# tzeitim/rogtk

Hardware: AMD Instinct MI355X
Metric: reads/s UMI score+cluster, 150 bp/12 bp UMI, 1→8 MI355X; % HBM roofline (higher is better)
Workload: dtype u32/f64

## Files before the change

rogtk_amd/csrc/cluster_kernels.hip:

```cpp
#include <hip/hip_ext.h>
#include <hipcub/hipcub.hpp>

#include <algorithm>
#include <cstdlib>
#include <map>
#include <mutex>

#include <atomic>
#include <thread>
#include <chrono>
#include <cstring>

#include "rogtk_internal.h"

namespace rogtk {
namespace {

constexpr int kBlock = 256;
constexpr int kMarkParts = 8;
constexpr int kMarkChunks = 256;
constexpr int kScanWords = 1024;
constexpr int kLocal8Words = 1024;
constexpr int kLocal8Cap = 8192;
constexpr int kLocal8BigCap = 16384;
// ... 1758 lines not shown
    if (rounds) {
        ++st.epoch;
        st.launched = launched;
        st.checked = checked;
        st.pending = true;
    }
    return ROGTK_OK;
}

int cluster_finish(const void* ws, hipStream_t s, int* redone) {
    if (redone) *redone = 0;
    std::lock_guard<std::mutex> lk(g_rs_mu);
    auto it = g_rs.find(ws);
    if (it == g_rs.end() || !it->second.pending) return ROGTK_OK;
    return finish_locked(ws, it->second, s, redone);
}

namespace {
int finish_locked(const void* ws, ResolveState& st, hipStream_t s, int* redone) {
    if (int rc = wait_published(st)) return rc;
    unsigned int* hflags = (unsigned int*)(st.hstats + kFlagsOff);
    const unsigned long long* hs = (const unsigned long long*)st.hstats;
    st.lcc_choice = hs[S_P0] == 8 ? (int)hs[S_LCAP] : 2;
    const bool redo = hs[S_REDO] != 0;
    const int scanned = st.launched + (st.checked ? 1 : 0);
    st.checked = false;
    if (!redo) {
        if (int z = first_zero(hflags, 0, scanned); z >= 0) {
            st.pending = false;
            st.deferred.on = false;
            st.rounds = z + 1;
            st.needed = st.rounds;
            return ROGTK_OK;
        }
    }
    if (redone) *redone = 1;
    WsPtrs p = ws_ptrs(st.cl, const_cast<uint8_t*>((const uint8_t*)ws));
    if (redo) {
        ProfScope prof(K_UNION, s);
        ROGTK_HIP_CHECK(hipMemsetAsync(p.stats + S_REDO, 0, 8, s));
        launch_local_cc(p.RT, st.cl.words, st.cl.L, p.f, p.UR, p.lroot, st.cl.rwords, st.cl.max_distinct, p.stats, s,
                        -1);
        ROGTK_HIP_CHECK(hipGetLastError());
        ROGTK_HIP_CHECK(hipMemsetAsync(p.flags, 0, kMaxRounds * sizeof(unsigned int), s));
        std::memset(hflags, 0, kMaxRounds * sizeof(unsigned int));
        st.launched = 0;
    }
    bool converged = false;
    while (!converged && st.launched < kMaxRounds) {
        const int to = std::min(st.launched + kRoundBatch, kMaxRounds);
        {
            ProfScope prof(K_UNION, s);
            if (int rc = enqueue_rounds(st.cl, p, st.launched, to, s)) return rc;
        }
        ROGTK_HIP_CHECK(hipMemcpyAsync(hflags + st.launched, p.flags + st.launched,
                                       (to - st.launched) * sizeof(unsigned int), hipMemcpyDeviceToHost, s));
        ROGTK_HIP_CHECK(hipStreamSynchronize(s));
        const int z = first_zero(hflags, st.launched, to);
        converged = z >= 0;
        if (converged) st.rounds = st.needed = z + 1;
        st.launched = to;
    }
    st.pending = false;
    ROGTK_REQUIRE(converged, ROGTK_E_HIP, "cluster: union rounds did not converge in %d rounds", kMaxRounds);
    if (int rc = enqueue_labels(st.cl, p, s, nullptr)) return rc;
    if (st.deferred.on) {
        st.deferred.on = false;
        return enqueue_assign(st.cl, p, st.word_labels ? 1 : st.exact ? 2 : 0, st.deferred.codes, st.deferred.regbits, st.deferred.n,
                              st.deferred.cid, s);
    }
    return ROGTK_OK;
}
}

int cluster_set_spec_rounds(int n) {
    ROGTK_REQUIRE(n >= 0 && n <= kMaxRounds, ROGTK_E_INVALID, "spec rounds %d outside 0..%d", n, kMaxRounds);
    g_spec_rounds.store(n == 0 ? kSpecRounds : n);
    g_spec_adaptive.store(n == 0);
    return ROGTK_OK;
}

int cluster_set_lookback_polls(int n) {
    ROGTK_REQUIRE(n >= -1, ROGTK_E_INVALID, "look-back polls %d < -1", n);
    g_lb_polls.store(n < 0 ? kLbMaxPolls : n);
    return ROGTK_OK;
}

int cluster_rounds(const void* ws, hipStream_t s, int* rounds) {
    if (int rc = cluster_finish(ws, s)) return rc;
    std::lock_guard<std::mutex> lk(g_rs_mu);
    auto it = g_rs.find(ws);
    *rounds = it == g_rs.end() ? 0 : it->second.rounds;
    return ROGTK_OK;
}

void cluster_release(const void* ws) {
    std::lock_guard<std::mutex> lk(g_rs_mu);
    auto it = g_rs.find(ws);
    if (it == g_rs.end()) return;
    if (it->second.hstats) {
        if (it->second.pending) (void)wait_published(it->second);
        hipHostFree(it->second.hstats);
    }
    g_rs.erase(it);
}

int launch_cluster_assign(const ClusterLayout& cl, const uint8_t* ws, const uint32_t* codes,
                          const uint64_t* regular_bits, int64_t n, uint32_t* cluster_id,
                          hipStream_t s, bool deferred) {
    if (!deferred)
        if (int rc = cluster_finish(ws, s)) return rc;
    WsPtrs p = ws_ptrs(cl, const_cast<uint8_t*>(ws));
    int wl = 0;
    {
        std::lock_guard<std::mutex> lk(g_rs_mu);
        auto it = g_rs.find(ws);
        if (it != g_rs.end()) {
            wl = it->second.word_labels ? 1 : it->second.exact ? 2 : 0;
            if (deferred && it->second.pending) {
                auto& d = it->second.deferred;
                d.on = true;
                d.codes = codes;
                d.regbits = regular_bits;
                d.n = n;
                d.cid = cluster_id;
            }
        }
    }
    return enqueue_assign(cl, p, wl, codes, regular_bits, n, cluster_id, s);
}

int cluster_assign_prepare(const ClusterLayout& cl, const uint8_t* ws, const uint32_t* codes,
                           const uint64_t* regular_bits, int64_t n, uint32_t* cluster_id, hipStream_t s,
                           bool deferred, AssignIn* a) {
    a->wlab = nullptr;
    a->wexc = nullptr;
    a->labelcode = nullptr;
    a->out = nullptr;
    if (!deferred)
        if (int rc = cluster_finish(ws, s)) return rc;
    bool wl = false;
    {
        std::lock_guard<std::mutex> lk(g_rs_mu);
        auto it = g_rs.find(ws);
        if (it != g_rs.end()) {
            wl = it->second.word_labels;
            if (deferred && it->second.pending) {
                auto& d = it->second.deferred;
                d.on = true;
                d.codes = codes;
                d.regbits = regular_bits;
                d.n = n;
                d.cid = cluster_id;
            }
        }
    }
    if (!wl || !cl.label_by_code) return ROGTK_OK;
    WsPtrs p = ws_ptrs(cl, const_cast<uint8_t*>(ws));
    a->wlab = p.wpref;
    a->wexc = p.G;
    a->labelcode = p.labelcode;
    a->out = cluster_id;
    return ROGTK_OK;
}

int launch_cluster_lookup(const ClusterLayout& cl, const uint8_t* ws, const uint64_t* q, int64_t nq, uint32_t* lab,
                          hipStream_t s) {
    if (nq <= 0) return ROGTK_OK;
    if (int rc = cluster_finish(ws, s)) return rc;
    WsPtrs p = ws_ptrs(cl, const_cast<uint8_t*>(ws));
    bool wl = false;
    {
        std::lock_guard<std::mutex> lk(g_rs_mu);
        auto it = g_rs.find(ws);
        if (it != g_rs.end()) wl = it->second.word_labels;
    }
    const uint32_t* wlab = wl ? p.wpref : nullptr;
    const uint64_t* wexc = wl ? p.G : nullptr;
    const int g = grid_for(nq, 4096);
    if (cl.label_by_code)
        hipLaunchKernelGGL(k_lookup<0>, dim3(g), dim3(kBlock), 0, s, q, nq, cl.nbits, p.labelcode, p.D, p.RT, wlab,
                           wexc, lab);
    else
        hipLaunchKernelGGL(k_lookup<1>, dim3(g), dim3(kBlock), 0, s, q, nq, cl.nbits, p.labelcode, p.ilab, p.RT, wlab,
                           wexc, lab);
    ROGTK_HIP_CHECK(hipGetLastError());
    return ROGTK_OK;
}

#ifndef ROGTK_ASSIGN_WGS
#define ROGTK_ASSIGN_WGS 2
#endif
#ifndef ROGTK_ASSIGN_G
#define ROGTK_ASSIGN_G 2
#endif
namespace {
int enqueue_assign(const ClusterLayout& cl, const WsPtrs& p, int labels, const uint32_t* codes,
                   const uint64_t* regular_bits, int64_t n, uint32_t* cluster_id, hipStream_t s) {
    if (n <= 0) return ROGTK_OK;
    const uint32_t* wlab = labels == 1 ? p.wpref : nullptr;
    const uint64_t* wexc = labels == 1 ? p.G : nullptr;
    ProfScope prof(K_ASSIGN, s, true);
    static const int64_t cap = [] {
        int dev = 0, cus = 0;
        if (hipGetDevice(&dev) != hipSuccess ||
            hipDeviceGetAttribute(&cus, hipDeviceAttributeMultiprocessorCount, dev) != hipSuccess || cus <= 0)
            cus = 256;
        return (int64_t)ROGTK_ASSIGN_WGS * cus;
    }();
    constexpr int kGroups = ROGTK_ASSIGN_G;
    const int g = grid_for((n + 4 * kGroups - 1) / (4 * kGroups), cap);
    if (labels == 2)
        hipExtLaunchKernelGGL((k_assign<2, kGroups>), dim3(g), dim3(kBlock), 0, s, prof.start(), prof.stop(), 0, codes,
                              regular_bits, n, p.labelcode, p.ilab, p.RT, wlab, wexc, cluster_id);
    else if (cl.label_by_code)
        hipExtLaunchKernelGGL((k_assign<0, kGroups>), dim3(g), dim3(kBlock), 0, s, prof.start(), prof.stop(), 0, codes,
                              regular_bits, n, p.labelcode, p.D, p.RT, wlab, wexc, cluster_id);
    else
        hipExtLaunchKernelGGL((k_assign<1, kGroups>), dim3(g), dim3(kBlock), 0, s, prof.start(), prof.stop(), 0, codes,
                              regular_bits, n, p.labelcode, p.ilab, p.RT, wlab, wexc, cluster_id);
    ROGTK_HIP_CHECK(hipGetLastError());
    return ROGTK_OK;
}
}



namespace {

constexpr int kPartBits = 8;
constexpr int kPartBlock = 512;

__global__ __launch_bounds__(kBlock) void k_mark_keys(const uint32_t* __restrict__ codes,
                                                      const uint64_t* __restrict__ regbits, int64_t n,
                                                      uint32_t* __restrict__ keys) {
    const int64_t i = (int64_t)blockIdx.x * kBlock + threadIdx.x;
    if (i >= n) return;
    const bool reg = (regbits[i >> 6] >> (i & 63)) & 1ull;
    keys[i] = reg ? codes[i] : 0xFFFFFFFFu;
}

__device__ int64_t wg_lower_bound(const uint32_t* __restrict__ a, int64_t n, uint64_t v) {
    int64_t lo = 0, hi = n;
    while (lo < hi) {
        const int64_t step = (hi - lo + kPartBlock - 1) / kPartBlock;
        const int64_t pos = lo + (int64_t)threadIdx.x * step;
        const bool less = pos < hi && (uint64_t)a[pos] < v;
        const int64_t cnt = __syncthreads_count(less);
        const int64_t nlo = cnt ? lo + (cnt - 1) * step + 1 : lo;
        const int64_t nhi = min(hi, lo + cnt * step);
        lo = nlo;
        hi = nhi;
    }
    return lo;
}

__global__ __launch_bounds__(kPartBlock) void k_part_bitmap(const uint32_t* __restrict__ sorted, int64_t n,
                                                            int two_l, uint64_t* __restrict__ bitmap) {
    extern __shared__ uint32_t lbits[];
    const int p = blockIdx.x;
    const int shift = two_l - kPartBits;
    const uint32_t pwords32 = (1u << shift) >> 5;
    for (uint32_t k = threadIdx.x; k < pwords32; k += kPartBlock) lbits[k] = 0;
    __shared__ int64_t range[2];
    const int64_t r0 = wg_lower_bound(sorted, n, (uint64_t)p << shift);
    const int64_t r1 = p + 1 == (1 << kPartBits) ? n : wg_lower_bound(sorted, n, (uint64_t)(p + 1) << shift);
    if (threadIdx.x == 0) {
        range[0] = r0;
        range[1] = r1;
    }
    __syncthreads();
    const uint32_t mask = (1u << shift) - 1u;
    constexpr int kUnroll = 8;
    const int64_t rend = range[1];
    for (int64_t i0 = range[0] + threadIdx.x; i0 < rend; i0 += (int64_t)kPartBlock * kUnroll) {
        uint32_t key[kUnroll];
#pragma unroll
        for (int u = 0; u < kUnroll; ++u) {
            const int64_t i = i0 + (int64_t)u * kPartBlock;
            key[u] = i < rend ? __builtin_nontemporal_load(sorted + i) : 0xFFFFFFFFu;
        }
#pragma unroll
        for (int u = 0; u < kUnroll; ++u) {
            if ((uint64_t)key[u] >> two_l) continue;
            const uint32_t c = key[u] & mask;
            atomicOr(&lbits[c >> 5], 1u << (c & 31));
        }
    }
    __syncthreads();
    uint64_t* out = bitmap + ((uint64_t)p << shift >> 6);
    for (uint32_t k = threadIdx.x; k < pwords32 / 2; k += kPartBlock)
        out[k] = (uint64_t)lbits[2 * k] | ((uint64_t)lbits[2 * k + 1] << 32);
}

#ifndef ROGTK_SLICE_BLOCK
#define ROGTK_SLICE_BLOCK 1024
#endif
constexpr int kSliceBlock = ROGTK_SLICE_BLOCK;
constexpr int kSliceChunks = 8;
#ifndef ROGTK_SLICE_LOG2
#define ROGTK_SLICE_LOG2 20
#endif
constexpr int kSliceLog2 = ROGTK_SLICE_LOG2;
constexpr int kSliceBits = 24 - kSliceLog2;
constexpr int kMaxSlices = 1 << kSliceBits;
constexpr int kBucketRows = 8192;
constexpr int kSegCap = kBucketRows * 4 / kMaxSlices;

__global__ __launch_bounds__(kSliceBlock) void k_slice_mark(const uint32_t* __restrict__ codes,
                                                            const uint64_t* __restrict__ regbits, int64_t n,
                                                            int slice_log2, int chunks, int64_t chunk_rows,
                                                            uint64_t* __restrict__ out, int64_t words,
                                                            const uint32_t* __restrict__ segs = nullptr,
                                                            const uint32_t* __restrict__ seglen = nullptr,
                                                            int nbuckets = 0, int bucket_rows = kBucketRows,
                                                            int seg_cap = kSegCap) {
    __shared__ uint32_t sbits[(1u << kSliceLog2) / 32];
    const int c = blockIdx.x % chunks, sl = blockIdx.x / chunks;
    const uint32_t sw32 = (1u << slice_log2) >> 5;
    for (uint32_t k = threadIdx.x; k < sw32; k += kSliceBlock) sbits[k] = 0;
    __syncthreads();
    const uint32_t smask = (1u << slice_log2) - 1u;
    int64_t r0 = (int64_t)c * chunk_rows, r1 = min(n, r0 + chunk_rows);
    if (segs) {
        const int b0 = (int)((int64_t)c * nbuckets / chunks), b1 = (int)((int64_t)(c + 1) * nbuckets / chunks);
        bool over = false;
        for (int b = b0 + (int)threadIdx.x; b < b1; b += kSliceBlock)
            over |= seglen[(int64_t)sl * nbuckets + b] > (uint32_t)seg_cap;
        r0 = (int64_t)b0 * bucket_rows;
        r1 = min(n, (int64_t)b1 * bucket_rows);
        if (!__syncthreads_or(over)) {
            constexpr int kSegInFlight = 8;
            constexpr int kWaves = kSliceBlock / 64;
            const int wave = threadIdx.x >> 6, lane = threadIdx.x & 63;
            for (int bb = b0 + wave; bb < b1; bb += kWaves * kSegInFlight) {
                uint32_t len[kSegInFlight];
                uint32_t mx = 0;
#pragma unroll
                for (int u = 0; u < kSegInFlight; ++u) {
                    const int b = bb + u * kWaves;
                    len[u] = b < b1 ? seglen[(int64_t)sl * nbuckets + b] : 0u;
                    mx = max(mx, len[u]);
                }
                for (uint32_t i = 4 * lane; i < mx; i += 256) {
                    uint4 v[kSegInFlight];
#pragma unroll
                    for (int u = 0; u < kSegInFlight; ++u) {
                        const uint32_t* seg = segs + ((int64_t)sl * nbuckets + bb + u * kWaves) * seg_cap;
                        v[u] = i < len[u] ? *reinterpret_cast<const uint4*>(seg + i) : make_uint4(0, 0, 0, 0);
                    }
#pragma unroll
                    for (int u = 0; u < kSegInFlight; ++u) {
                        const uint32_t cc[4] = {v[u].x, v[u].y, v[u].z, v[u].w};
#pragma unroll
                        for (int k = 0; k < 4; ++k)
                            if (i + k < len[u]) {
                                const uint32_t b2 = cc[k] & smask;
                                atomicOr(&sbits[b2 >> 5], 1u << (b2 & 31));
                            }
                    }
                }
            }
            r1 = r0;
        }
    }
    constexpr int kSliceUnroll = 8;
    constexpr int64_t kStep = 4 * (int64_t)kSliceBlock;
    for (int64_t rb = r0 + 4 * (int64_t)threadIdx.x; rb < r1; rb += kStep * kSliceUnroll) {
        uint4 v[kSliceUnroll];
        uint32_t reg[kSliceUnroll];
#pragma unroll
        for (int u = 0; u < kSliceUnroll; ++u) {
            const int64_t r = rb + u * kStep;
            reg[u] = 0;
            v[u] = make_uint4(0, 0, 0, 0);
            if (r + 4 <= r1) {
                v[u] = *reinterpret_cast<const uint4*>(codes + r);
                reg[u] = regbits ? (uint32_t)(regbits[r >> 6] >> (r & 63)) & 0xFu : 0xFu;
            } else if (r < r1) {
                v[u].x = codes[r];
                if (r + 1 < r1) v[u].y = codes[r + 1];
                if (r + 2 < r1) v[u].z = codes[r + 2];
                reg[u] = (regbits ? (uint32_t)(regbits[r >> 6] >> (r & 63)) & 0xFu : 0xFu) &
                         ((1u << (uint32_t)(r1 - r)) - 1u);
            }
        }
#pragma unroll
        for (int u = 0; u < kSliceUnroll; ++u) {
            const uint32_t cc[4] = {v[u].x, v[u].y, v[u].z, v[u].w};
#pragma unroll
            for (int k = 0; k < 4; ++k)
                if (((reg[u] >> k) & 1u) && (cc[k] >> slice_log2) == (uint32_t)sl) {
                    const uint32_t b = cc[k] & smask;
                    atomicOr(&sbits[b >> 5], 1u << (b & 31));
                }
        }
    }
    __syncthreads();
    uint64_t* o = out + (int64_t)c * words + (((int64_t)sl << slice_log2) >> 6);
    for (uint32_t k = threadIdx.x; k < sw32 / 2; k += kSliceBlock)
        o[k] = (uint64_t)sbits[2 * k] | ((uint64_t)sbits[2 * k + 1] << 32);
}

constexpr int kBucketThreads = 1024;
template <int kBucketRows, int kBucketThreads>
__global__ __launch_bounds__(kBucketThreads) void k_slice_bucket(const uint32_t* __restrict__ codes,
                                                         const uint64_t* __restrict__ regbits, int64_t n,
                                                         int slice_log2, int nslices, uint32_t* __restrict__ segs,
                                                         uint32_t* __restrict__ seglen, int nbuckets) {
    __shared__ unsigned int cnt[kMaxSlices], lbase[kMaxSlices + 1];
    constexpr int kSegCap = kBucketRows * 4 / kMaxSlices;
    __shared__ uint32_t stage[kBucketRows];
    const int t = threadIdx.x, lane = t & 63;
    if (t < kMaxSlices) cnt[t] = 0;
    __syncthreads();
    const int64_t row0 = (int64_t)blockIdx.x * kBucketRows;
    constexpr int kPer = kBucketRows / kBucketThreads / 4;
    uint32_t key[kPer * 4];
    uint32_t val[kPer * 4];
    uint32_t regs[kPer];
#pragma unroll
    for (int u = 0; u < kPer; ++u) {
        const int64_t r = row0 + 4 * ((int64_t)u * kBucketThreads + t);
        uint4 v = make_uint4(0, 0, 0, 0);
        uint32_t reg = 0;
        if (r + 4 <= n) {
            v = *reinterpret_cast<const uint4*>(codes + r);
            reg = regbits ? (uint32_t)(regbits[r >> 6] >> (r & 63)) & 0xFu : 0xFu;
        } else if (r < n) {
            v.x = codes[r];
            if (r + 1 < n) v.y = codes[r + 1];
            if (r + 2 < n) v.z = codes[r + 2];
            reg = (regbits ? (uint32_t)(regbits[r >> 6] >> (r & 63)) & 0xFu : 0xFu) & ((1u << (uint32_t)(n - r)) - 1u);
        }
        val[4 * u] = v.x;
        val[4 * u + 1] = v.y;
        val[4 * u + 2] = v.z;
        val[4 * u + 3] = v.w;
        regs[u] = reg;
    }
#pragma unroll
    for (int u = 0; u < kPer; ++u) {
#pragma unroll
        for (int k = 0; k < 4; ++k) {
            const uint32_t sl = val[4 * u + k] >> slice_log2;
            const bool ok = ((regs[u] >> k) & 1u) && sl < (uint32_t)nslices;
            uint64_t peers = __ballot(ok);
#pragma unroll
            for (int bit = 0; bit < kSliceBits; ++bit) {
                const uint64_t b = __ballot((sl >> bit) & 1u);
                peers &= ((sl >> bit) & 1u) ? b : ~b;
            }
            const int leader = peers ? __ffsll((long long)peers) - 1 : 0;
            unsigned int base = 0;
            if (ok && lane == leader) base = atomicAdd(&cnt[sl], (unsigned int)__popcll(peers));
            base = __shfl(base, leader);
            key[4 * u + k] = ok ? (sl << 16) | (base + (uint32_t)__popcll(peers & ((1ull << lane) - 1ull))) : kNone;
        }
    }
    __syncthreads();
    if (t < nslices) seglen[(int64_t)t * nbuckets + blockIdx.x] = cnt[t];
    if (t == 0) {
        unsigned int acc = 0;
        for (int k = 0; k < nslices; ++k) {
            lbase[k] = acc;
            acc += cnt[k];
        }
        lbase[nslices] = acc;
    }
    __syncthreads();
#pragma unroll
    for (int u = 0; u < kPer * 4; ++u) {
        const uint32_t kk = key[u];
        if (kk != kNone) stage[lbase[kk >> 16] + (kk & 0xFFFFu)] = val[u];
    }
    __syncthreads();
    const unsigned int total = lbase[nslices];
    for (unsigned int i = t; i < total; i += kBucketThreads) {
        const uint32_t c = stage[i];
        const uint32_t sl = c >> slice_log2;
        if (cnt[sl] <= (unsigned int)kSegCap) segs[((int64_t)sl * nbuckets + blockIdx.x) * kSegCap + (i - lbase[sl])] = c;
    }
}

__global__ __launch_bounds__(kBlock) void k_or_partials(const uint64_t* __restrict__ partials, int chunks,
                                                        int64_t words, uint64_t* __restrict__ out) {
    for (int64_t w = (int64_t)blockIdx.x * kBlock + threadIdx.x; w < words; w += (int64_t)gridDim.x * kBlock) {
        uint64_t v = 0;
        for (int c = 0; c < chunks; ++c) v |= __builtin_nontemporal_load(partials + (int64_t)c * words + w);
        out[w] = v;
    }
}

inline int slice_chunks(int64_t n) { return n >= (1 << 20) ? kSliceChunks : 1; }
inline bool slice_segments(int64_t n) { return n >= (1 << 20); }
inline int slices_of(int L) { return 1 << (2 * L - std::min(2 * L, kSliceLog2)); }
inline int64_t seg_buckets(int64_t n) { return (n + kBucketRows - 1) / kBucketRows; }
inline int64_t seg_bytes(int64_t n) {
    return ((int64_t)kMaxSlices * seg_buckets(n) * kSegCap * 4) + ((int64_t)kMaxSlices * seg_buckets(n) * 4 + 255) / 256 * 256;
}
inline bool slice_buckets_on() {
    static const bool on = [] {
        const char* e = getenv("ROGTK_SLICE_BUCKETS");
        return !(e && e[0] == '0');
    }();
    return on;
}

size_t part_sort_temp(int64_t n) {
    size_t tb = 0;
    hipcub::DeviceRadixSort::SortKeys(nullptr, tb, (const uint32_t*)nullptr, (uint32_t*)nullptr, (int)n, 0, 8);
    return tb;
}

}

namespace {
std::atomic<int> g_mark_method{0};
bool use_slices(int L) {
    const int m = g_mark_method.load();
    return L <= 12 && m != 1;
}
}

int cluster_set_mark_method(int m) {
    ROGTK_REQUIRE(m >= 0 && m <= 2, ROGTK_E_INVALID, "mark method %d outside 0..2", m);
    g_mark_method.store(m);
    return ROGTK_OK;
}

int cluster_mark_bitmap_temp(int64_t n, int L, int64_t* bytes) {
    ROGTK_REQUIRE(L >= 7 && L <= 13, ROGTK_E_UNSUPPORTED, "mark_bitmap needs umi_len 7..13, got %d", L);
    ROGTK_REQUIRE(n >= 0 && n < ((int64_t)1 << 31), ROGTK_E_INVALID, "n outside 0..2^31-1");
    const int64_t nn = std::max<int64_t>(n, 1);
    const int64_t sort_bytes = 2 * ((nn * 4 + 255) / 256 * 256) + (int64_t)part_sort_temp(nn) + 256;
    const int64_t words = ((int64_t)1 << (2 * L)) / 64;
    int64_t slice_bytes = 0;
    if (L <= 12 && slice_segments(nn)) {
        slice_bytes = slice_chunks(nn) > 1 ? (int64_t)slice_chunks(nn) * words * 8 : 0;
        if (slices_of(L) > 1) slice_bytes += seg_bytes(nn);
    }
    *bytes = std::max(sort_bytes, slice_bytes);
    return ROGTK_OK;
}

int launch_cluster_mark_bitmap(const uint32_t* codes, const uint64_t* regular_bits, int64_t n, int L,
                               uint64_t* bitmap, void* temp, int64_t temp_bytes, hipStream_t s) {
    return launch_cluster_mark_phase(codes, regular_bits, n, L, bitmap, temp, temp_bytes, 0, s);
}

int launch_cluster_mark_phase(const uint32_t* codes, const uint64_t* regular_bits, int64_t n, int L,
                              uint64_t* bitmap, void* temp, int64_t temp_bytes, int phase, hipStream_t s) {
    ROGTK_REQUIRE(phase >= 0 && phase <= 2, ROGTK_E_INVALID, "mark_bitmap: phase %d", phase);
    int64_t need = 0;
    if (int rc = cluster_mark_bitmap_temp(n, L, &need)) return rc;
    ROGTK_REQUIRE((temp || n == 0) && temp_bytes >= need, ROGTK_E_INVALID, "temp_bytes %lld < %lld", (long long)temp_bytes,
                  (long long)need);
    ProfScope prof(K_MARK, s);
    const int two_l = 2 * L;
    if (n == 0) {
        if (phase != 1) ROGTK_HIP_CHECK(hipMemsetAsync(bitmap, 0, ((size_t)1 << two_l) / 8, s));
        return ROGTK_OK;
    }
    ROGTK_REQUIRE(((uintptr_t)codes & 15u) == 0, ROGTK_E_INVALID, "mark_bitmap: codes must be 16-byte aligned");
    if (use_slices(L)) {
        const int slog = std::min(two_l, kSliceLog2);
        const int slices = 1 << (two_l - slog);
        const int chunks = slice_chunks(n);
        int64_t chunk_rows = (n + chunks - 1) / chunks;
        chunk_rows = (chunk_rows + 3) / 4 * 4;
        const int64_t words = ((int64_t)1 << two_l) / 64;
        uint64_t* dst = chunks > 1 ? (uint64_t*)temp : bitmap;
        const uint32_t* segs = nullptr;
        uint32_t* seglen = nullptr;
        const int nb = (int)seg_buckets(n);
        if (slice_segments(n) && slices > 1 && slices <= kMaxSlices && slice_buckets_on()) {
            segs = (const uint32_t*)((uint8_t*)temp + (chunks > 1 ? (int64_t)chunks * words * 8 : 0));
            seglen = (uint32_t*)((uint8_t*)segs + (int64_t)kMaxSlices * nb * kSegCap * 4);
            if (phase != 2)
                ROGTK_TIMED_LAUNCH(K_K_SLICE_BUCKET, (k_slice_bucket<kBucketRows, kBucketThreads>), dim3((unsigned)nb),
                                   dim3(kBucketThreads), 0, s, codes, regular_bits, n, slog, slices, (uint32_t*)segs,
                                   seglen, nb);
        }
        if (phase == 1) {
            ROGTK_HIP_CHECK(hipGetLastError());
            return ROGTK_OK;
        }
        ROGTK_TIMED_LAUNCH(K_K_SLICE_MARK, k_slice_mark, dim3((unsigned)(slices * chunks)), dim3(kSliceBlock), 0, s, codes, regular_bits,
                           n, slog, chunks, chunk_rows, dst, words, segs, (const uint32_t*)seglen, nb, kBucketRows, kSegCap);
        if (chunks > 1)
            ROGTK_TIMED_LAUNCH(K_K_OR_PARTIALS, k_or_partials, dim3(grid_for(words, 4096)), dim3(kBlock), 0, s, dst, chunks, words,
                               bitmap);
        ROGTK_HIP_CHECK(hipGetLastError());
        return ROGTK_OK;
    }
    if (phase == 1) return ROGTK_OK;
    const int64_t slab = (n * 4 + 255) / 256 * 256;
    uint32_t* keys_in = (uint32_t*)temp;
    uint32_t* keys_out = (uint32_t*)((uint8_t*)temp + slab);
    void* cub = (uint8_t*)temp + 2 * slab;
    const uint32_t* src = codes;
    if (regular_bits) {
        hipLaunchKernelGGL(k_mark_keys, dim3((unsigned)((n + kBlock - 1) / kBlock)), dim3(kBlock), 0, s, codes,
                           regular_bits, n, keys_in);
        src = keys_in;
    }
    size_t tb = part_sort_temp(n);
    ROGTK_HIP_CHECK(hipcub::DeviceRadixSort::SortKeys(cub, tb, src, keys_out, (int)n, two_l - kPartBits, two_l, s));
    const size_t lds = ((size_t)1 << (two_l - kPartBits)) / 8;
    hipLaunchKernelGGL(k_part_bitmap, dim3(1u << kPartBits), dim3(kPartBlock), lds, s, keys_out, n, two_l, bitmap);
    ROGTK_HIP_CHECK(hipGetLastError());
    return ROGTK_OK;
}

}

#ifdef ROGTK_LCC_TIMING
extern "C" int rogtk_debug_lcc_clock(unsigned long long* out8) {
    if (hipMemcpyFromSymbol(out8, HIP_SYMBOL(rogtk::g_lcc_clk), 64) != hipSuccess) return 1;
    const unsigned long long z[8] = {0, 0, 0, 0, 0, 0, 0, 0};
    return hipMemcpyToSymbol(HIP_SYMBOL(rogtk::g_lcc_clk), z, 64) == hipSuccess ? 0 : 1;
}
#endif
```

Baseline: 36.75 billion.

## Replace capped slice segments with compact 16-bit bucketed runs and per-slice mark

```diff
diff --git a/rogtk_amd/csrc/cluster_kernels.hip b/rogtk_amd/csrc/cluster_kernels.hip
--- a/rogtk_amd/csrc/cluster_kernels.hip
+++ b/rogtk_amd/csrc/cluster_kernels.hip
@@ -2084,68 +2084,18 @@
 #define ROGTK_SLICE_LOG2 20
 #endif
 constexpr int kSliceLog2 = ROGTK_SLICE_LOG2;
-constexpr int kSliceBits = 24 - kSliceLog2;
-constexpr int kMaxSlices = 1 << kSliceBits;
-constexpr int kBucketRows = 8192;
-constexpr int kSegCap = kBucketRows * 4 / kMaxSlices;
 
 __global__ __launch_bounds__(kSliceBlock) void k_slice_mark(const uint32_t* __restrict__ codes,
                                                             const uint64_t* __restrict__ regbits, int64_t n,
                                                             int slice_log2, int chunks, int64_t chunk_rows,
-                                                            uint64_t* __restrict__ out, int64_t words,
-                                                            const uint32_t* __restrict__ segs = nullptr,
-                                                            const uint32_t* __restrict__ seglen = nullptr,
-                                                            int nbuckets = 0, int bucket_rows = kBucketRows,
-                                                            int seg_cap = kSegCap) {
+                                                            uint64_t* __restrict__ out, int64_t words) {
     __shared__ uint32_t sbits[(1u << kSliceLog2) / 32];
     const int c = blockIdx.x % chunks, sl = blockIdx.x / chunks;
     const uint32_t sw32 = (1u << slice_log2) >> 5;
     for (uint32_t k = threadIdx.x; k < sw32; k += kSliceBlock) sbits[k] = 0;
     __syncthreads();
     const uint32_t smask = (1u << slice_log2) - 1u;
-    int64_t r0 = (int64_t)c * chunk_rows, r1 = min(n, r0 + chunk_rows);
-    if (segs) {
-        const int b0 = (int)((int64_t)c * nbuckets / chunks), b1 = (int)((int64_t)(c + 1) * nbuckets / chunks);
-        bool over = false;
-        for (int b = b0 + (int)threadIdx.x; b < b1; b += kSliceBlock)
-            over |= seglen[(int64_t)sl * nbuckets + b] > (uint32_t)seg_cap;
-        r0 = (int64_t)b0 * bucket_rows;
-        r1 = min(n, (int64_t)b1 * bucket_rows);
-        if (!__syncthreads_or(over)) {
-            constexpr int kSegInFlight = 8;
-            constexpr int kWaves = kSliceBlock / 64;
-            const int wave = threadIdx.x >> 6, lane = threadIdx.x & 63;
-            for (int bb = b0 + wave; bb < b1; bb += kWaves * kSegInFlight) {
-                uint32_t len[kSegInFlight];
-                uint32_t mx = 0;
-#pragma unroll
-                for (int u = 0; u < kSegInFlight; ++u) {
-                    const int b = bb + u * kWaves;
-                    len[u] = b < b1 ? seglen[(int64_t)sl * nbuckets + b] : 0u;
-                    mx = max(mx, len[u]);
-                }
-                for (uint32_t i = 4 * lane; i < mx; i += 256) {
-                    uint4 v[kSegInFlight];
-#pragma unroll
-                    for (int u = 0; u < kSegInFlight; ++u) {
-                        const uint32_t* seg = segs + ((int64_t)sl * nbuckets + bb + u * kWaves) * seg_cap;
-                        v[u] = i < len[u] ? *reinterpret_cast<const uint4*>(seg + i) : make_uint4(0, 0, 0, 0);
-                    }
-#pragma unroll
-                    for (int u = 0; u < kSegInFlight; ++u) {
-                        const uint32_t cc[4] = {v[u].x, v[u].y, v[u].z, v[u].w};
-#pragma unroll
-                        for (int k = 0; k < 4; ++k)
-                            if (i + k < len[u]) {
-                                const uint32_t b2 = cc[k] & smask;
-                                atomicOr(&sbits[b2 >> 5], 1u << (b2 & 31));
-                            }
-                    }
-                }
-            }
-            r1 = r0;
-        }
-    }
+    const int64_t r0 = (int64_t)c * chunk_rows, r1 = min(n, r0 + chunk_rows);
     constexpr int kSliceUnroll = 8;
     constexpr int64_t kStep = 4 * (int64_t)kSliceBlock;
     for (int64_t rb = r0 + 4 * (int64_t)threadIdx.x; rb < r1; rb += kStep * kSliceUnroll) {
@@ -2184,26 +2134,48 @@
         o[k] = (uint64_t)sbits[2 * k] | ((uint64_t)sbits[2 * k + 1] << 32);
 }
 
-constexpr int kBucketThreads = 1024;
-template <int kBucketRows, int kBucketThreads>
-__global__ __launch_bounds__(kBucketThreads) void k_slice_bucket(const uint32_t* __restrict__ codes,
-                                                         const uint64_t* __restrict__ regbits, int64_t n,
-                                                         int slice_log2, int nslices, uint32_t* __restrict__ segs,
-                                                         uint32_t* __restrict__ seglen, int nbuckets) {
-    __shared__ unsigned int cnt[kMaxSlices], lbase[kMaxSlices + 1];
-    constexpr int kSegCap = kBucketRows * 4 / kMaxSlices;
-    __shared__ uint32_t stage[kBucketRows];
+__global__ __launch_bounds__(kBlock) void k_or_partials(const uint64_t* __restrict__ partials, int chunks,
+                                                        int64_t words, uint64_t* __restrict__ out) {
+    for (int64_t w = (int64_t)blockIdx.x * kBlock + threadIdx.x; w < words; w += (int64_t)gridDim.x * kBlock) {
+        uint64_t v = 0;
+        for (int c = 0; c < chunks; ++c) v |= __builtin_nontemporal_load(partials + (int64_t)c * words + w);
+        out[w] = v;
+    }
+}
+
+#ifndef ROGTK_B16_ROWS
+#define ROGTK_B16_ROWS 8192
+#endif
+#ifndef ROGTK_S16_BLOCK
+#define ROGTK_S16_BLOCK 512
+#endif
+constexpr int kS16Log2 = 16;
+constexpr int kS16MaxSlices = 1 << (24 - kS16Log2);
+constexpr int kB16Rows = ROGTK_B16_ROWS;
+constexpr int kB16Threads = 1024;
+constexpr int kB16Stride = kB16Rows + 8 * kS16MaxSlices;
+constexpr int kS16Block = ROGTK_S16_BLOCK;
+constexpr int kS16InFlight = 8;
+static_assert(kB16Stride < 65536 && kB16Rows % (4 * kB16Threads) == 0, "(start, length) are uint16 pairs");
+
+template <int kRows, int kThreads>
+__global__ __launch_bounds__(kThreads) void k_slice_bucket16(const uint32_t* __restrict__ codes,
+                                                             const uint64_t* __restrict__ regbits, int64_t n,
+                                                             int nslices, uint16_t* __restrict__ blocks,
+                                                             uint32_t* __restrict__ table, int nbuckets) {
+    __shared__ unsigned int cnt[kS16MaxSlices], start[kS16MaxSlices], total;
+    __shared__ __attribute__((aligned(16))) uint16_t stage[kRows + 8 * kS16MaxSlices];
     const int t = threadIdx.x, lane = t & 63;
-    if (t < kMaxSlices) cnt[t] = 0;
-    __syncthreads();
-    const int64_t row0 = (int64_t)blockIdx.x * kBucketRows;
-    constexpr int kPer = kBucketRows / kBucketThreads / 4;
+    if (t < kS16MaxSlices) cnt[t] = 0;
+    __syncthreads();
+    const int64_t row0 = (int64_t)blockIdx.x * kRows;
+    constexpr int kPer = kRows / kThreads / 4;
     uint32_t key[kPer * 4];
     uint32_t val[kPer * 4];
     uint32_t regs[kPer];
 #pragma unroll
     for (int u = 0; u < kPer; ++u) {
-        const int64_t r = row0 + 4 * ((int64_t)u * kBucketThreads + t);
+        const int64_t r = row0 + 4 * ((int64_t)u * kThreads + t);
         uint4 v = make_uint4(0, 0, 0, 0);
         uint32_t reg = 0;
         if (r + 4 <= n) {
@@ -2225,62 +2197,97 @@
     for (int u = 0; u < kPer; ++u) {
 #pragma unroll
         for (int k = 0; k < 4; ++k) {
-            const uint32_t sl = val[4 * u + k] >> slice_log2;
+            const uint32_t sl = val[4 * u + k] >> kS16Log2;
             const bool ok = ((regs[u] >> k) & 1u) && sl < (uint32_t)nslices;
-            uint64_t peers = __ballot(ok);
-#pragma unroll
-            for (int bit = 0; bit < kSliceBits; ++bit) {
-                const uint64_t b = __ballot((sl >> bit) & 1u);
-                peers &= ((sl >> bit) & 1u) ? b : ~b;
-            }
-            const int leader = peers ? __ffsll((long long)peers) - 1 : 0;
-            unsigned int base = 0;
-            if (ok && lane == leader) base = atomicAdd(&cnt[sl], (unsigned int)__popcll(peers));
-            base = __shfl(base, leader);
-            key[4 * u + k] = ok ? (sl << 16) | (base + (uint32_t)__popcll(peers & ((1ull << lane) - 1ull))) : kNone;
-        }
-    }
-    __syncthreads();
-    if (t < nslices) seglen[(int64_t)t * nbuckets + blockIdx.x] = cnt[t];
-    if (t == 0) {
-        unsigned int acc = 0;
-        for (int k = 0; k < nslices; ++k) {
-            lbase[k] = acc;
-            acc += cnt[k];
-        }
-        lbase[nslices] = acc;
-    }
-    __syncthreads();
+            key[4 * u + k] = ok ? (sl << 16) | atomicAdd(&cnt[sl], 1u) : kNone;
+        }
+    }
+    __syncthreads();
+    if (t < 64) {
+        unsigned int pre[4], sum = 0;
+#pragma unroll
+        for (int j = 0; j < 4; ++j) {
+            pre[j] = sum;
+            sum += (cnt[4 * t + j] + 7u) & ~7u;
+        }
+        unsigned int inc = sum;
+#pragma unroll
+        for (int d = 1; d < 64; d <<= 1) {
+            const unsigned int o = __shfl_up(inc, d);
+            if (lane >= d) inc += o;
+        }
+#pragma unroll
+        for (int j = 0; j < 4; ++j) start[4 * t + j] = inc - sum + pre[j];
+        if (t == 63) total = inc;
+    }
+    __syncthreads();
+    if (t < nslices) table[(int64_t)t * nbuckets + blockIdx.x] = start[t] | (cnt[t] << 16);
 #pragma unroll
     for (int u = 0; u < kPer * 4; ++u) {
         const uint32_t kk = key[u];
-        if (kk != kNone) stage[lbase[kk >> 16] + (kk & 0xFFFFu)] = val[u];
-    }
-    __syncthreads();
-    const unsigned int total = lbase[nslices];
-    for (unsigned int i = t; i < total; i += kBucketThreads) {
-        const uint32_t c = stage[i];
-        const uint32_t sl = c >> slice_log2;
-        if (cnt[sl] <= (unsigned int)kSegCap) segs[((int64_t)sl * nbuckets + blockIdx.x) * kSegCap + (i - lbase[sl])] = c;
-    }
-}
-
-__global__ __launch_bounds__(kBlock) void k_or_partials(const uint64_t* __restrict__ partials, int chunks,
-                                                        int64_t words, uint64_t* __restrict__ out) {
-    for (int64_t w = (int64_t)blockIdx.x * kBlock + threadIdx.x; w < words; w += (int64_t)gridDim.x * kBlock) {
-        uint64_t v = 0;
-        for (int c = 0; c < chunks; ++c) v |= __builtin_nontemporal_load(partials + (int64_t)c * words + w);
-        out[w] = v;
-    }
-}
+        if (kk != kNone) stage[start[kk >> 16] + (kk & 0xFFFFu)] = (uint16_t)val[u];
+    }
+    __syncthreads();
+    const uint4* s4 = reinterpret_cast<const uint4*>(stage);
+    uint4* o4 = reinterpret_cast<uint4*>(blocks + (int64_t)blockIdx.x * kB16Stride);
+    for (unsigned int i = t; i < total / 8; i += kThreads) o4[i] = s4[i];
+}
+
+template <int kThreads, int kG>
+__global__ __launch_bounds__(kThreads) void k_slice_mark16(const uint16_t* __restrict__ blocks,
+                                                           const uint32_t* __restrict__ table, int nbuckets,
+                                                           uint64_t* __restrict__ bitmap) {
+    __shared__ uint32_t sbits[(1u << kS16Log2) / 32];
+    constexpr int kWords32 = (1 << kS16Log2) / 32;
+    constexpr int kGroups = kThreads / kG, kU = kS16InFlight;
+    const int t = threadIdx.x, g = t / kG, gl = t % kG, sl = blockIdx.x;
+    for (int k = t; k < kWords32; k += kThreads) sbits[k] = 0;
+    __syncthreads();
+    const uint32_t* tab = table + (int64_t)sl * nbuckets;
+    uint32_t te[kU];
+#pragma unroll
+    for (int u = 0; u < kU; ++u) te[u] = g + u * kGroups < nbuckets ? tab[g + u * kGroups] : 0u;
+    for (int bb = g; bb < nbuckets; bb += kGroups * kU) {
+        uint32_t nx[kU], mx = 0;
+#pragma unroll
+        for (int u = 0; u < kU; ++u) {
+            const int b = bb + (kU + u) * kGroups;
+            nx[u] = b < nbuckets ? tab[b] : 0u;
+            mx = max(mx, te[u] >> 16);
+        }
+        for (uint32_t i = 8 * gl; i < mx; i += 8 * kG) {
+            uint4 v[kU];
+#pragma unroll
+            for (int u = 0; u < kU; ++u) {
+                const uint16_t* run = blocks + (int64_t)(bb + u * kGroups) * kB16Stride + (te[u] & 0xFFFFu);
+                v[u] = i < (te[u] >> 16) ? *reinterpret_cast<const uint4*>(run + i) : make_uint4(0, 0, 0, 0);
+            }
+#pragma unroll
+            for (int u = 0; u < kU; ++u) {
+                const uint32_t w[4] = {v[u].x, v[u].y, v[u].z, v[u].w};
+                const uint32_t len = te[u] >> 16;
+#pragma unroll
+                for (int k = 0; k < 8; ++k)
+                    if (i + k < len) {
+                        const uint32_t c = (w[k >> 1] >> (16 * (k & 1))) & 0xFFFFu;
+                        atomicOr(&sbits[c >> 5], 1u << (c & 31));
+                    }
+            }
+        }
+#pragma unroll
+        for (int u = 0; u < kU; ++u) te[u] = nx[u];
+    }
+    __syncthreads();
+    uint64_t* o = bitmap + (int64_t)sl * (kWords32 / 2);
+    for (int k = t; k < kWords32 / 2; k += kThreads) o[k] = (uint64_t)sbits[2 * k] | ((uint64_t)sbits[2 * k + 1] << 32);
+}
+
+inline int64_t b16_buckets(int64_t n) { return (n + kB16Rows - 1) / kB16Rows; }
+inline int64_t b16_block_bytes(int64_t n) { return b16_buckets(n) * kB16Stride * 2; }
+inline int64_t b16_bytes(int64_t n) { return b16_block_bytes(n) + (int64_t)kS16MaxSlices * b16_buckets(n) * 4; }
+inline bool slice16_applies(int64_t n, int L) { return L >= 9 && L <= 12 && n >= (1 << 20); }
 
 inline int slice_chunks(int64_t n) { return n >= (1 << 20) ? kSliceChunks : 1; }
-inline bool slice_segments(int64_t n) { return n >= (1 << 20); }
-inline int slices_of(int L) { return 1 << (2 * L - std::min(2 * L, kSliceLog2)); }
-inline int64_t seg_buckets(int64_t n) { return (n + kBucketRows - 1) / kBucketRows; }
-inline int64_t seg_bytes(int64_t n) {
-    return ((int64_t)kMaxSlices * seg_buckets(n) * kSegCap * 4) + ((int64_t)kMaxSlices * seg_buckets(n) * 4 + 255) / 256 * 256;
-}
 inline bool slice_buckets_on() {
     static const bool on = [] {
         const char* e = getenv("ROGTK_SLICE_BUCKETS");
@@ -2317,11 +2324,8 @@
     const int64_t nn = std::max<int64_t>(n, 1);
     const int64_t sort_bytes = 2 * ((nn * 4 + 255) / 256 * 256) + (int64_t)part_sort_temp(nn) + 256;
     const int64_t words = ((int64_t)1 << (2 * L)) / 64;
-    int64_t slice_bytes = 0;
-    if (L <= 12 && slice_segments(nn)) {
-        slice_bytes = slice_chunks(nn) > 1 ? (int64_t)slice_chunks(nn) * words * 8 : 0;
-        if (slices_of(L) > 1) slice_bytes += seg_bytes(nn);
-    }
+    int64_t slice_bytes = L <= 12 && slice_chunks(nn) > 1 ? (int64_t)slice_chunks(nn) * words * 8 : 0;
+    if (slice16_applies(nn, L)) slice_bytes = std::max(slice_bytes, b16_bytes(nn));
     *bytes = std::max(sort_bytes, slice_bytes);
     return ROGTK_OK;
 }
@@ -2345,6 +2349,28 @@
         return ROGTK_OK;
     }
     ROGTK_REQUIRE(((uintptr_t)codes & 15u) == 0, ROGTK_E_INVALID, "mark_bitmap: codes must be 16-byte aligned");
+    if (use_slices(L) && slice16_applies(n, L) && slice_buckets_on()) {
+        const int slices = 1 << (two_l - kS16Log2);
+        const int nb = (int)b16_buckets(n);
+        uint16_t* blocks = (uint16_t*)temp;
+        uint32_t* table = (uint32_t*)((uint8_t*)temp + b16_block_bytes(n));
+        if (phase != 2)
+            ROGTK_TIMED_LAUNCH(K_K_SLICE_BUCKET, (k_slice_bucket16<kB16Rows, kB16Threads>), dim3((unsigned)nb),
+                               dim3(kB16Threads), 0, s, codes, regular_bits, n, slices, blocks, table, nb);
+        if (phase != 1) {
+            if (slices >= 256)
+                ROGTK_TIMED_LAUNCH(K_K_SLICE_MARK, (k_slice_mark16<kS16Block, 8>), dim3((unsigned)slices), dim3(kS16Block),
+                                   0, s, (const uint16_t*)blocks, (const uint32_t*)table, nb, bitmap);
+            else if (slices >= 64)
+                ROGTK_TIMED_LAUNCH(K_K_SLICE_MARK, (k_slice_mark16<kS16Block, 32>), dim3((unsigned)slices), dim3(kS16Block),
+                                   0, s, (const uint16_t*)blocks, (const uint32_t*)table, nb, bitmap);
+            else
+                ROGTK_TIMED_LAUNCH(K_K_SLICE_MARK, (k_slice_mark16<kS16Block, 64>), dim3((unsigned)slices), dim3(kS16Block),
+                                   0, s, (const uint16_t*)blocks, (const uint32_t*)table, nb, bitmap);
+        }
+        ROGTK_HIP_CHECK(hipGetLastError());
+        return ROGTK_OK;
+    }
     if (use_slices(L)) {
         const int slog = std::min(two_l, kSliceLog2);
         const int slices = 1 << (two_l - slog);
@@ -2353,23 +2379,9 @@
         chunk_rows = (chunk_rows + 3) / 4 * 4;
         const int64_t words = ((int64_t)1 << two_l) / 64;
         uint64_t* dst = chunks > 1 ? (uint64_t*)temp : bitmap;
-        const uint32_t* segs = nullptr;
-        uint32_t* seglen = nullptr;
-        const int nb = (int)seg_buckets(n);
-        if (slice_segments(n) && slices > 1 && slices <= kMaxSlices && slice_buckets_on()) {
-            segs = (const uint32_t*)((uint8_t*)temp + (chunks > 1 ? (int64_t)chunks * words * 8 : 0));
-            seglen = (uint32_t*)((uint8_t*)segs + (int64_t)kMaxSlices * nb * kSegCap * 4);
-            if (phase != 2)
-                ROGTK_TIMED_LAUNCH(K_K_SLICE_BUCKET, (k_slice_bucket<kBucketRows, kBucketThreads>), dim3((unsigned)nb),
-                                   dim3(kBucketThreads), 0, s, codes, regular_bits, n, slog, slices, (uint32_t*)segs,
-                                   seglen, nb);
-        }
-        if (phase == 1) {
-            ROGTK_HIP_CHECK(hipGetLastError());
-            return ROGTK_OK;
-        }
+        if (phase == 1) return ROGTK_OK;
         ROGTK_TIMED_LAUNCH(K_K_SLICE_MARK, k_slice_mark, dim3((unsigned)(slices * chunks)), dim3(kSliceBlock), 0, s, codes, regular_bits,
-                           n, slog, chunks, chunk_rows, dst, words, segs, (const uint32_t*)seglen, nb, kBucketRows, kSegCap);
+                           n, slog, chunks, chunk_rows, dst, words);
         if (chunks > 1)
             ROGTK_TIMED_LAUNCH(K_K_OR_PARTIALS, k_or_partials, dim3(grid_for(words, 4096)), dim3(kBlock), 0, s, dst, chunks, words,
                                bitmap);
```

After: 38.30 billion, median of 6. +4.2%, better.
